# amathislab/HOISDF

Hardware: AMD Instinct MI355X
Metric: samples/sec (img + 2048 SDF queries) fwd+bwd at 1/2/4/8 MI355X (higher is better)
Workload: dtype f32 (emulated contractions, f32 accumulate, f16x2 form: operands as scaled hi + lo f16 pieces x 3 products - 22 operand bits, one power-of-two scale per ROW of a linear layer's row operand, per (sample, head) of the attention operands, per weight matrix; the attention backward's dS as three pieces x

## Files before the change

hoisdf_amd/csrc/attention_emu.h:

```cpp
#pragma once
#include "common.h"

namespace hoisdf {
namespace emu_attn {

typedef float f32x16 __attribute__((ext_vector_type(16)));
typedef float f32x4 __attribute__((ext_vector_type(4)));
typedef float f32x2 __attribute__((ext_vector_type(2)));
typedef __bf16 bf16x8 __attribute__((ext_vector_type(8)));
typedef __bf16 bf16x4 __attribute__((ext_vector_type(4)));
typedef __bf16 bf16x2 __attribute__((ext_vector_type(2)));
typedef _Float16 f16x8 __attribute__((ext_vector_type(8)));
typedef _Float16 f16x2 __attribute__((ext_vector_type(2)));
typedef unsigned int u32x4 __attribute__((ext_vector_type(4)));
typedef unsigned int u32x2 __attribute__((ext_vector_type(2)));
typedef short s16x4 __attribute__((ext_vector_type(4)));

constexpr int D = 64;
constexpr float LN2 = 0.6931471805599453f;

struct EmuAttn {
  const __bf16 *q[3];
  const __bf16 *k[3];
  const __bf16 *v[3], *vt[3];
  const __bf16 *d[3];
  const float* lse_in; const float* delta;
  float* out; float* lse; float* dq_part; float* dk; float* dv;
  int ldo, ldk, ldv;
  int B, H, Lq, Lk, Lqp, Lkp, kv_len;
  float drop_p, inv_keep;
  uint32_t thresh;
  uint64_t seed;
  const uint32_t *q_hm, *k_hm, *v_hm, *d_hm;
  float* dq_scale;
  uint32_t* mag;
};

__device__ __forceinline__ bool emu_block(int nx, int nbh, int& tile, int& bh) {
  const int L = blockIdx.x, slot = L >> 3;
  bh = (slot / nx) * 8 + (L & 7);
  tile = slot % nx;
  return bh < nbh;
}

}

int attention_bwd4_emu_launch(const emu_attn::EmuAttn& a, hipStream_t st);
int attention_bwd4h_emu_launch(const emu_attn::EmuAttn& a, hipStream_t st);
}
```

hoisdf_amd/csrc/attention_emu.hip:

```cpp
#include "attention_emu.h"

namespace hoisdf {
using namespace emu_attn;

namespace {
constexpr int RP = 72;
constexpr int TPH = 36;
constexpr int ROWS_T = 32 * RP;
constexpr int TRN_T = 64 * TPH;
constexpr float QS2 = 0.125f * 1.4426950408889634f;
#define CR(r, h) (((r) & 3) + 8 * ((r) >> 2) + 4 * (h))
#define MB(a, b, c) __builtin_amdgcn_mfma_f32_32x32x16_bf16((a), (b), (c), 0, 0, 0)
#define MB6(acc, x0, x1, x2, y0, y1, y2) \
  do {                                   \
    acc = MB(x2, y0, acc);               \
    acc = MB(x0, y2, acc);               \
    acc = MB(x1, y1, acc);               \
    acc = MB(x1, y0, acc);               \
    acc = MB(x0, y1, acc);               \
    acc = MB(x0, y0, acc);               \
  } while (0)

#define SPLIT1(x, i)                             \
  do {                                           \
// ... 505 lines not shown
  HOISDF_REQUIRE(workspace_bytes >= need, HOISDF_ERR_WORKSPACE, "attention_fwd_bf16x2: workspace %ld < %ld bytes", workspace_bytes, need);
  hipStream_t st = as_stream(stream);
  __bf16* w = reinterpret_cast<__bf16*>(workspace);
  const QkvPlaneSet s = carve_qkv(w, B, H, Lq, Lk, false, true, 2);
  if (int rc = convert_qkv(q, ldq, k, ldk, v, ldv, B, H, Lq, Lk, s, st)) return rc;
  EmuAttn a = emu_args(B, H, Lq, Lk, kv_len, 0.f, 0);
  for (int i = 0; i < 2; ++i) { a.q[i] = s.q.r[i]; a.k[i] = s.k.r[i]; a.vt[i] = s.v.t[i]; }
  a.out = o; a.lse = nullptr; a.ldo = ldo;
  const dim3 fgrid(cdiv(Lq, 128) * 8 * cdiv(B * H, 8));
  hipLaunchKernelGGL((emu_attn_fwd2_kernel<false, 2, false>), fgrid, dim3(256), 0, st, a);
  return check_launch("attention_fwd_bf16x2");
}

void hoisdf::attention_emu_plane_targets(void* workspace, int B, int H, int Lq, int Lk, int keep, QkvPlanes& qp, QkvPlanes& kvp) {
  const QkvPlaneSet s = fwd_planes(workspace, B, H, Lq, Lk, keep);
  qp = QkvPlanes{}; kvp = QkvPlanes{};
  qp.on = kvp.on = 1; qp.H = kvp.H = H; qp.E = kvp.E = H * 64; qp.qscale = kvp.qscale = QS2;
  qp.L = Lq; qp.Lp = (int)pad128(Lq); kvp.L = Lk; kvp.Lp = (int)pad128(Lk);
  for (int i = 0; i < 3; ++i) {
    qp.r[0][i] = s.q.r[i];
    kvp.r[1][i] = s.k.r[i]; kvp.r[2][i] = s.v.r[i]; kvp.vt[i] = s.v.t[i];
    if (Lq == Lk) { kvp.r[0][i] = s.q.r[i]; qp.r[1][i] = s.k.r[i]; qp.r[2][i] = s.v.r[i]; qp.vt[i] = s.v.t[i]; }
  }
}

int hoisdf::attention_fwd_emu_planes(float* o, int ldo, float* lse, int B, int H, int Lq, int Lk, int kv_len, float drop_p,
                                     uint64_t seed, void* workspace, int keep, void* stream, uint32_t* o_mag) {
  HOISDF_REQUIRE(o && workspace && ldo >= H * 64 && (ldo & 3) == 0 && (((uintptr_t)o | (uintptr_t)workspace) & 15) == 0 && B > 0 &&
                     H > 0 && Lq > 0 && Lk > 0 && kv_len > 0 && kv_len <= Lk && drop_p >= 0.f && drop_p < 1.f,
                 HOISDF_ERR_INVALID, "attention_fwd_emu_planes: bad arguments");
  return fwd_over_planes(o, ldo, lse, B, H, Lq, Lk, kv_len, drop_p, seed, workspace, keep, as_stream(stream), o_mag);
}

extern "C" long hoisdf_attention_bwd_emu_workspace(int B, int H, int Lq, int Lk, int kept) {
  if (B <= 0 || H <= 0 || Lq <= 0 || Lk <= 0) return 0;
  const size_t q = plane_elems(B, H, pad128(Lq)), k = plane_elems(B, H, pad128(Lk));
  size_t bytes = 3 * q * sizeof(__bf16) + (size_t)cdiv(Lk, 128) * B * H * Lq * 64 * sizeof(float);
  if (!kept) bytes += (3 * q + 6 * k) * sizeof(__bf16);
  return (long)bytes;
}

extern "C" int hoisdf_attention_bwd_emu(const float* q, int ldq, const float* k, int ldk, const float* v, int ldv, const float* o,
                                        int ldo, const float* dout, int lddo, const float* lse, float* delta, float* dq, float* dk,
                                        float* dv, int B, int H, int Lq, int Lk, int kv_len, float drop_p, uint64_t seed,
                                        const void* fwd_workspace, void* workspace, long workspace_bytes, void* stream) {
  return attention_bwd_emu_mag(q, ldq, k, ldk, v, ldv, o, ldo, dout, lddo, lse, delta, dq, dk, dv, B, H, Lq, Lk, kv_len, drop_p, seed,
                               fwd_workspace, workspace, workspace_bytes, nullptr, stream, nullptr, nullptr, nullptr, nullptr);
}
extern "C" int hoisdf_attention_bwd_emu_mag(const float* q, int ldq, const float* k, int ldk, const float* v, int ldv, const float* o,
                                            int ldo, const float* dout, int lddo, const float* lse, float* delta, float* dq, float* dk,
                                            float* dv, int B, int H, int Lq, int Lk, int kv_len, float drop_p, uint64_t seed,
                                            const void* fwd_workspace, void* workspace, long workspace_bytes, const uint32_t* q_mag,
                                            const uint32_t* k_mag, const uint32_t* v_mag, const uint32_t* do_mag, uint32_t* g_mag, void* stream) {
  HOISDF_REQUIRE(q_mag && k_mag && v_mag && do_mag, HOISDF_ERR_INVALID, "attention_bwd_emu_mag: the head magnitudes of q, k, v and of dout are required");
  return attention_bwd_emu_mag(q, ldq, k, ldk, v, ldv, o, ldo, dout, lddo, lse, delta, dq, dk, dv, B, H, Lq, Lk, kv_len, drop_p, seed,
                               fwd_workspace, workspace, workspace_bytes, g_mag, stream, q_mag, k_mag, v_mag, do_mag);
}
int hoisdf::attention_bwd_emu_mag(const float* q, int ldq, const float* k, int ldk, const float* v, int ldv, const float* o, int ldo,
                                  const float* dout, int lddo, const float* lse, float* delta, float* dq, float* dk, float* dv, int B,
                                  int H, int Lq, int Lk, int kv_len, float drop_p, uint64_t seed, const void* fwd_workspace,
                                  void* workspace, long workspace_bytes, uint32_t* g_mag, void* stream, const uint32_t* q_hm,
                                  const uint32_t* k_hm, const uint32_t* v_hm, const uint32_t* do_hm) {
  const bool h2 = q_hm && k_hm && v_hm && do_hm;
  HOISDF_REQUIRE(h2 || (!q_hm && !k_hm && !v_hm && !do_hm), HOISDF_ERR_INVALID, "attention_bwd_emu: head magnitudes of all of q, k, v, dout or of none");
  HOISDF_REQUIRE(!g_mag || Lq == Lk, HOISDF_ERR_INVALID, "attention_bwd_emu: one row-magnitude array for dq, dk, dv needs Lq == Lk");
  HOISDF_REQUIRE(!h2 || drop_p < 0.75f, HOISDF_ERR_INVALID, "attention_bwd_emu (f16x2 form): drop_p = %f, must be below 0.75 (as in the forward)", drop_p);
  if (int rc = check_emu(fwd_workspace && !q ? o : q, fwd_workspace && !k ? o : k, fwd_workspace && !v ? o : v, ldq, ldk, ldv, B, H, Lq,
                         Lk, kv_len, drop_p, "attention_bwd_emu")) return rc;
  HOISDF_REQUIRE(o && dout && lse && delta && dq && dk && dv && workspace, HOISDF_ERR_INVALID, "attention_bwd_emu: null pointer");
  HOISDF_REQUIRE(ldo >= H * 64 && lddo >= H * 64 && ((ldo | lddo) & 3) == 0 &&
                     (((uintptr_t)o | (uintptr_t)dout | (uintptr_t)dq | (uintptr_t)dk | (uintptr_t)dv | (uintptr_t)workspace |
                       (uintptr_t)fwd_workspace) & 15) == 0,
                 HOISDF_ERR_INVALID, "attention_bwd_emu: bad leading dims / alignment");
  const long need = hoisdf_attention_bwd_emu_workspace(B, H, Lq, Lk, fwd_workspace ? 1 : 0);
  HOISDF_REQUIRE(workspace_bytes >= need, HOISDF_ERR_WORKSPACE, "attention_bwd_emu: workspace %ld < %ld bytes", workspace_bytes, need);
  hipStream_t st = as_stream(stream);
  __bf16* w = reinterpret_cast<__bf16*>(workspace);
  const Planes pd = carve(w, plane_elems(B, H, pad128(Lq)), true, false);
  float* part = reinterpret_cast<float*>(w);
  w += (size_t)cdiv(Lk, 128) * B * H * Lq * 64 * 2;
  QkvPlaneSet s;
  if (fwd_workspace) {
    __bf16* f = reinterpret_cast<__bf16*>(const_cast<void*>(fwd_workspace));
    s = carve_qkv(f, B, H, Lq, Lk, true, true);
  } else {
    s = carve_qkv(w, B, H, Lq, Lk, true, false);
    if (int rc = convert_qkv(q, ldq, k, ldk, v, ldv, B, H, Lq, Lk, s, st, q_hm, k_hm, v_hm)) return rc;
  }
  if (int rc = convert(dout, lddo, Lq, (int)pad128(Lq), B, H, 1.f, pd, st, do_hm)) return rc;
  const long ng = (long)B * Lq * H;
  hipLaunchKernelGGL(emu_attn_delta_kernel, dim3((unsigned)((ng * 16 + 255) / 256)), dim3(256), 0, st, o, ldo, dout, lddo, delta, B, H, Lq);
  if (int rc = check_launch("attention_emu_delta")) return rc;
  EmuAttn a = emu_args(B, H, Lq, Lk, kv_len, drop_p, seed);
  for (int i = 0; i < 3; ++i) { a.q[i] = s.q.r[i]; a.k[i] = s.k.r[i]; a.v[i] = s.v.r[i]; a.d[i] = pd.r[i]; }
  a.lse_in = lse; a.delta = delta; a.dq_part = part; a.dk = dk; a.dv = dv; a.ldk = ldk; a.ldv = ldv; a.mag = g_mag;
  if (h2) {
    a.q_hm = q_hm; a.k_hm = k_hm; a.v_hm = v_hm; a.d_hm = do_hm;
    a.dq_scale = reinterpret_cast<float*>(pd.r[2]);
  }
  if (int rc = h2 ? attention_bwd4h_emu_launch(a, st) : attention_bwd4_emu_launch(a, st)) return rc;
  const long n4 = (long)B * H * Lq * 16;
  hipLaunchKernelGGL(emu_attn_dq_reduce_kernel, dim3((unsigned)((n4 + 255) / 256)), dim3(256), 0, st, part, cdiv(kv_len, 128), dq, ldq,
                     B, H, Lq, g_mag, (const float*)(h2 ? a.dq_scale : nullptr));
  return check_launch("attention_bwd_emu dq reduce");
}
```

hoisdf_amd/csrc/attention_emu_bwd4.inc:

```

namespace hoisdf {
namespace {
constexpr int NPL = B4_NPL;
constexpr int QD_PLANE = 32 * 64;
constexpr int QD_BUF = 2 * NPL * QD_PLANE;
constexpr int TT_PLANE = 128 * 32;
constexpr int TT_BUF = 3 * TT_PLANE;
constexpr int X_BUF = 2 * 32 * 64;
constexpr int TT0 = 3 * QD_BUF;
constexpr int X0_BYTES = (3 * QD_BUF + 2 * TT_BUF) * 2;
constexpr int ST0_BYTES = X0_BYTES + 2 * X_BUF * 4;
constexpr unsigned B4_LDS_BYTES = ST0_BYTES + 3 * 64 * 4;

__device__ __forceinline__ int qd_swz(int r) { return ((r >> 1) & 3) | ((((r >> 1) ^ (r >> 3)) & 1) << 2); }
__device__ __forceinline__ int qd_off(int r, int ch) { return r * 64 + ((ch ^ qd_swz(r)) << 3); }

__device__ __forceinline__ bf16x8 tr8(const __bf16* lo, const __bf16* hi) {
  const s16x4 x = __builtin_amdgcn_ds_read_tr16_b64_v4i16((s16x4 __attribute__((address_space(3)))*)(lo));
  const s16x4 y = __builtin_amdgcn_ds_read_tr16_b64_v4i16((s16x4 __attribute__((address_space(3)))*)(hi));
  return __builtin_bit_cast(bf16x8, __builtin_shufflevector(x, y, 0, 1, 2, 3, 4, 5, 6, 7));
}
}

template <bool DROP>
__global__ __launch_bounds__(256, 1) void B4_KERNEL(EmuAttn a) {
  extern __shared__ __attribute__((aligned(16))) __bf16 lds[];
  float* const xbuf = reinterpret_cast<float*>(reinterpret_cast<char*>(lds) + X0_BYTES);
  float* const stats = reinterpret_cast<float*>(reinterpret_cast<char*>(lds) + ST0_BYTES);
  const int tid = threadIdx.x, lane = tid & 63, wave = tid >> 6;
  const int c = lane & 31, h = lane >> 5, jq = lane & 15, b1 = (jq >> 3) & 1;
  int ktile, bh;
  const int nkb = (a.Lk + 127) / 128;
  if (!emu_block(nkb, a.B * a.H, ktile, bh)) return;
  const int b = bh / a.H, head = bh - b * a.H;
  const int key = ktile * 128 + wave * 32 + c;
  const bool kvalid = key < a.kv_len;
  const int nq = ktile * 128 < a.kv_len ? (a.Lq + 31) / 32 : 0;
  const int dhalf = wave & 1, khalf = wave >> 1;
  B4_SCALES

  bf16x8 kf[4][NPL], vf[4][NPL], ktf[4][NPL];
  {
    const size_t ro = ((size_t)bh * a.Lkp + key) * D;
#pragma unroll
    for (int p = 0; p < NPL; ++p)
#pragma unroll
      for (int j = 0; j < 4; ++j) {
        kf[j][p] = *reinterpret_cast<const bf16x8*>(a.k[p] + ro + 16 * j + 8 * h);
        vf[j][p] = *reinterpret_cast<const bf16x8*>(a.v[p] + ro + 16 * j + 8 * h);
      }
    const size_t ko = ((size_t)bh * a.Lkp + ktile * 128 + 64 * khalf + 8 * h) * D + 32 * dhalf + c;
#pragma unroll
    for (int p = 0; p < NPL; ++p)
#pragma unroll
      for (int ks = 0; ks < 4; ++ks) {
        bf16x8 t;
#pragma unroll
        for (int i = 0; i < 8; ++i)
          t[i] = ktile * 128 + 64 * khalf + 16 * ks + 8 * h + i < a.kv_len ? a.k[p][ko + (size_t)(16 * ks + i) * D] : (__bf16)0.f;
        ktf[ks][p] = t;
      }
  }
#pragma unroll
  for (int p = 0; p < NPL; ++p)
#pragma unroll
    for (int j = 0; j < 4; ++j) {
      asm volatile("" : "+a"(kf[j][p]));
// ... 16 lines not shown
#pragma unroll
    for (int e = 0; e < 2; ++e) trb[e] = (4 * h + (jq >> 2)) * 64 + ((e ^ b1) << 5) + (low2 << 3) + (jq & 1) * 4;
  }
  int tqb[2];
#pragma unroll
  for (int s2 = 0; s2 < 2; ++s2) {
    const int kr = 64 * khalf + 8 * h + 4 * s2 + (jq >> 2);
    tqb[s2] = kr * 32 + (((4 * (c >> 4) + (jq & 3)) ^ ((kr >> 1) & 7)) << 2);
  }
  const int tw0 = (32 * wave + c) * 32 + ((h ^ ((c >> 1) & 7)) << 2);
  const int xw0 = khalf * 2048 + c * 64 + (8 * dhalf << 2) + ((h ^ (c & 7)) << 2);
  const int xr0 = (8 * wave + (lane >> 4)) * 64 + (((lane & 15) ^ (lane >> 4)) << 2);
  const int xr1 = (xr0 + 256) ^ 16;
  const int st_o = qd_off(tid >> 3, tid & 7);

  u32x4 sg[2 * NPL];
  float rstat = 0.f;
  const size_t rowbase = (size_t)bh * a.Lqp * D;
  const __bf16* const qb0 = a.q[0] + rowbase; const __bf16* const qb1 = a.q[1] + rowbase; const __bf16* const qb2 = a.q[2] + rowbase;
  const __bf16* const db0 = a.d[0] + rowbase; const __bf16* const db1 = a.d[1] + rowbase; const __bf16* const db2 = a.d[2] + rowbase;
  unsigned goff = (unsigned)((tid >> 3) * D + (tid & 7) * 8);
  const float* const stat_src = (tid < 32 ? a.lse_in : a.delta) + (size_t)bh * a.Lq;
#define B4_LOADP(i_) do { sg[i_] = *reinterpret_cast<const u32x4*>(((i_) == 0 ? qb0 : (i_) == 1 ? qb1 : (i_) == NPL ? db0 : (i_) == NPL + 1 ? db1 : (i_) == 2 ? qb2 : db2) + goff); } while (0)
#define B4_LOADS(QT_, GHOST_)                                                                                          \
  do {                                                                                                                 \
    if (tid < 64) {                                                                                                    \
      const int q_ = (QT_) * 32 + (tid & 31);                                                                          \
      rstat = (q_ < a.Lq && !(GHOST_)) ? stat_src[q_] : (tid < 32 ? INFINITY : 0.f);                                   \
    }                                                                                                                  \
  } while (0)
#define B4_STOREP(i_, BUF_) do { *reinterpret_cast<u32x4*>(lds + (BUF_) + (i_) * QD_PLANE + st_o) = sg[i_]; } while (0)
#define B4_STORES(SB_) do { if (tid < 64) stats[(SB_) + tid] = rstat; } while (0)

  float* const part = a.dq_part + ((size_t)ktile * a.B * a.H + bh) * a.Lq * D;
  if (nq > 0) {
#pragma unroll
    for (int pt = 0; pt < 2; ++pt) {
      const int qt = min(pt, nq - 1);
      goff = (unsigned)(qt * 32 * D + (tid >> 3) * D + (tid & 7) * 8);
#pragma unroll
      for (int i = 0; i < 2 * NPL; ++i) B4_LOADP(i);
      B4_LOADS(qt, pt >= nq);
#pragma unroll
      for (int i = 0; i < 2 * NPL; ++i) B4_STOREP(i, pt * QD_BUF);
      B4_STORES(pt * 64);
    }
    int qt_next = min(2, nq - 1);
    goff = (unsigned)(qt_next * 32 * D + (tid >> 3) * D + (tid & 7) * 8);
#pragma unroll
    for (int i = 0; i < 2 * NPL; ++i) B4_LOADP(i);
    B4_LOADS(qt_next, 2 >= nq);
    __syncthreads();

    int qd_cur = 0, qd_nxt = QD_BUF, qd_fre = 2 * QD_BUF;
    int st_cur = 0, st_nxt = 64, st_fre = 128;
    int tt_w = TT0, tt_r = TT0 + TT_BUF;
    int x_a = 0, x_b = X_BUF;
    uint32_t hb = 0;
    const uint32_t dthr = a.thresh & 0xffff0000u;
    const int hsh = (key & 1) ? 0 : 16;
    B4_FORM_STATE
    if (DROP) hb = drop_rowkey(a.seed, (uint32_t)(bh * a.Lq + 4 * h)) + (uint32_t)(key >> 1) * 0x9E3779B9U + B4_HB_PAIR;

    f32x16 s, dp, dq;
    f32x4 xo0[2], xo1[2];
    bf16x8 fr[2][NPL];
    u32x4 pwv[NPL][2], gwv[3][2];
    f32x2 pe[8], pd[8], xx[8], ff[8];
    float dsc[16], lq[16], dl[16];
#pragma unroll
    for (int r = 0; r < 16; ++r) dsc[r] = 1.f;
#pragma unroll
    for (int p = 0; p < 3; ++p)
#pragma unroll
      for (int i = 0; i < 2; ++i) { if (p < NPL) pwv[p][i] = u32x4{0u, 0u, 0u, 0u}; gwv[p][i] = u32x4{0u, 0u, 0u, 0u}; }

#define MFMA_SP(acc_, a_, b_) asm volatile(B4_MFMA " %0, %1, %2, %0" : "+v"(acc_) : "v"(a_), "a"(b_))
#define MFMA_SP0(acc_, a_, b_) asm volatile(B4_MFMA " %0, %1, %2, 0" : "=&v"(acc_) : "v"(a_), "a"(b_))
#define MFMA_Q(acc_, a_, b_) asm volatile(B4_MFMA " %0, %1, %2, %0" : "+v"(acc_) : "a"(a_), "v"(b_))
#define MFMA_Q0(acc_, a_, b_) asm volatile(B4_MFMA " %0, %1, %2, 0" : "=&v"(acc_) : "a"(a_), "v"(b_))
#define MFMA_VK(acc_, a_, b_) asm volatile(B4_MFMA " %0, %1, %2, %0" : "+a"(acc_) : "v"(a_), "v"(b_))
#define FRQ(p_, j_) (*reinterpret_cast<const bf16x8*>(lds + qd_cur + aoff[j_] + (p_) * QD_PLANE))
#define FRD(p_, j_) (*reinterpret_cast<const bf16x8*>(lds + qd_cur + aoff[j_] + (NPL + (p_)) * QD_PLANE))
#define FRQN(p_, j_) (*reinterpret_cast<const bf16x8*>(lds + qd_nxt + aoff[j_] + (p_) * QD_PLANE))
#define FRDN(p_, j_) (*reinterpret_cast<const bf16x8*>(lds + qd_nxt + aoff[j_] + (NPL + (p_)) * QD_PLANE))
#define FRA(pl_, jj_, mt_) tr8(lds + qd_cur + trb[(mt_)] + (pl_) * QD_PLANE + (16 * (jj_)) * 64, \
                               lds + qd_cur + trb[(mt_) ^ 1] + (pl_) * QD_PLANE + (16 * (jj_) + 8) * 64)
#define FRT(p_, ks_) tr8(lds + tt_r + tqb[0] + (p_) * TT_PLANE + (16 * (ks_)) * 32, lds + tt_r + tqb[1] + (p_) * TT_PLANE + (16 * (ks_)) * 32)
#define PWF(p_, jj_) __builtin_bit_cast(bf16x8, pwv[p_][jj_])
#define GWF(p_, jj_) __builtin_bit_cast(bf16x8, gwv[p_][jj_])
#define PIN2(x_) asm volatile("" : "+v"(x_))
#define XOL(i_)                                                                                                        \
  do {                                                                                                                 \
    xo0[i_] = *reinterpret_cast<const f32x4*>(xbuf + x_a + ((i_) ? xr1 : xr0));                                        \
    xo1[i_] = *reinterpret_cast<const f32x4*>(xbuf + x_a + 2048 + ((i_) ? xr1 : xr0));                                 \
  } while (0)
#define XOS(i_)                                                                                                        \
  do {                                                                                                                 \
    const int q_ = (t - 2) * 32 + 8 * wave + 4 * (i_) + (lane >> 4);                                                   \
    if (t >= 2 && q_ < a.Lq) *reinterpret_cast<f32x4*>(part + (unsigned)(q_ * D + 4 * (lane & 15))) = xo0[i_] + xo1[i_]; \
  } while (0)
#define CRC(r_) (((r_) & 3) + 8 * ((r_) >> 2))
#define PB(q_)                                                                                                         \
  do {                                                                                                                 \
    _Pragma("unroll") for (int i_ = 0; i_ < 2; ++i_) {                                                                 \
      const int m_ = 2 * (q_) + i_;                                                                                    \
      pd[m_] = DROP ? f32x2{pe[m_].x * dsc[2 * m_], pe[m_].y * dsc[2 * m_ + 1]} : pe[m_];                              \
      const uint32_t w_ = cvt2(pd[m_]);                                                                                \
      pwv[0][m_ >> 2][m_ & 3] = w_;                                                                                    \
      PIN2(pwv[0][m_ >> 2][m_ & 3]);                                                                                   \
    }                                                                                                                  \
  } while (0)
#define PC(q_)                                                                                                         \
  do {                                                                                                                 \
    _Pragma("unroll") for (int i_ = 0; i_ < 2; ++i_) {                                                                 \
      const int m_ = 2 * (q_) + i_;                                                                                    \
      xx[m_] = pd[m_] - unpack2(pwv[0][m_ >> 2][m_ & 3]);                                                              \
      PIN2(xx[m_]);                                                                                                    \
    }                                                                                                                  \
  } while (0)
#define QB(q_)                                                                                                         \
  do {                                                                                                                 \
    _Pragma("unroll") for (int i_ = 0; i_ < 2; ++i_) {                                                                 \
      const int m_ = 2 * (q_) + i_;                                                                                    \
      xx[m_] = xx[m_] - unpack2(gwv[0][m_ >> 2][m_ & 3]);                                                              \
      PIN2(xx[m_]);                                                                                                    \
    }                                                                                                                  \
  } while (0)
#define QC(q_)                                                                                                         \
  do {                                                                                                                 \
    _Pragma("unroll") for (int i_ = 0; i_ < 2; ++i_) {                                                                 \
      const int m_ = 2 * (q_) + i_;                                                                                    \
      const uint32_t w_ = cvt2(xx[m_]);                                                                                \
// ... 33 lines not shown
      B4_ITER();
      { const int t_ = qd_cur; qd_cur = qd_nxt; qd_nxt = qd_fre; qd_fre = t_; }
      { const int t_ = st_cur; st_cur = st_nxt; st_nxt = st_fre; st_fre = t_; }
      { const int t_ = tt_w; tt_w = tt_r; tt_r = t_; }
      { const int t_ = x_a; x_a = x_b; x_b = t_; }
      __syncthreads();
    }
    {
      const int t = nq + 1;
      XOL(0); XOL(1);
      XOS(0); XOS(1);
    }
  }
  uint32_t gmax = 0u;
  if (key < a.Lk) {
    float* pk = a.dk + ((size_t)b * a.Lk + key) * a.ldk + head * D;
    float* pv = a.dv + ((size_t)b * a.Lk + key) * a.ldv + head * D;
#pragma unroll
    for (int mt = 0; mt < 2; ++mt)
#pragma unroll
      for (int g = 0; g < 4; ++g) {
        const float zk = kvalid ? dk_scale : 0.f, zv = kvalid ? dv_scale : 0.f;
        const float4 gk = make_float4(dk[mt][4 * g] * zk, dk[mt][4 * g + 1] * zk, dk[mt][4 * g + 2] * zk, dk[mt][4 * g + 3] * zk);
        const float4 gv = make_float4(dv[mt][4 * g] * zv, dv[mt][4 * g + 1] * zv, dv[mt][4 * g + 2] * zv, dv[mt][4 * g + 3] * zv);
        *reinterpret_cast<float4*>(pk + 32 * mt + 8 * g + 4 * h) = gk;
        *reinterpret_cast<float4*>(pv + 32 * mt + 8 * g + 4 * h) = gv;
        gmax = max(gmax, max(mag_bits4(gk), mag_bits4(gv)));
      }
  }
  if (a.mag) {
    gmax = max(gmax, (uint32_t)__shfl_xor((int)gmax, 32, 64));
    if (h == 0 && key < a.Lk) atomicMax(a.mag + (size_t)b * a.Lk + key, gmax);
  }
}

int B4_LAUNCH(const EmuAttn& a, hipStream_t st) {
  static bool attr_set = false;
  if (!attr_set) {
    const void* ks[2] = {reinterpret_cast<const void*>(B4_KERNEL<true>), reinterpret_cast<const void*>(B4_KERNEL<false>)};
    for (const void* k : ks)
      if (hipFuncSetAttribute(k, hipFuncAttributeMaxDynamicSharedMemorySize, (int)B4_LDS_BYTES) != hipSuccess) {
        set_error("attention_bwd_emu" B4_WHO ": cannot raise the dynamic LDS limit to %u bytes", B4_LDS_BYTES);
        return HOISDF_ERR_LAUNCH;
      }
    attr_set = true;
  }
  const dim3 grid(cdiv(a.Lk, 128) * 8 * cdiv(a.B * a.H, 8));
  if (a.drop_p > 0.f) hipLaunchKernelGGL((B4_KERNEL<true>), grid, dim3(256), B4_LDS_BYTES, st, a);
  else hipLaunchKernelGGL((B4_KERNEL<false>), grid, dim3(256), B4_LDS_BYTES, st, a);
  return check_launch("attention_bwd_emu (" B4_TAG ")");
}

}
```

hoisdf_amd/csrc/attn_bwd4_phase.inc:

```
#define BWD4_ITER()                                                                \
  do {                                                                             \
    MFMA_SP0(s, fr[0][0], kf[0][2]); XOL(0); SB();                                 \
    MFMA_SP(s, fr[0][2], kf[0][0]); fr[1][0] = FRQ(0, 1); XOL(1); SB();            \
    MFMA_SP(s, fr[0][1], kf[0][1]); fr[1][1] = FRQ(1, 1); SB();                    \
    MFMA_SP(s, fr[0][0], kf[0][1]); fr[1][2] = FRQ(2, 1); SB();                    \
    MFMA_SP(s, fr[0][1], kf[0][0]); STQ(0); SB();                                  \
    MFMA_SP(s, fr[0][0], kf[0][0]); STQ(1); SB();                                  \
    MFMA_SP(s, fr[1][0], kf[1][2]); STQ(2); SB();                                  \
    MFMA_SP(s, fr[1][2], kf[1][0]); fr[0][0] = FRQ(0, 2); SB();                    \
    MFMA_SP(s, fr[1][1], kf[1][1]); fr[0][1] = FRQ(1, 2); SB();                    \
    MFMA_SP(s, fr[1][0], kf[1][1]); fr[0][2] = FRQ(2, 2); SB();                    \
    MFMA_SP(s, fr[1][1], kf[1][0]); STQ(3); SB();                                  \
    MFMA_SP(s, fr[1][0], kf[1][0]); STQ(4); SB();                                  \
    MFMA_SP(s, fr[0][0], kf[2][2]); STQ(5); SB();                                  \
    MFMA_SP(s, fr[0][2], kf[2][0]); fr[1][0] = FRQ(0, 3); SB();                    \
    MFMA_SP(s, fr[0][1], kf[2][1]); fr[1][1] = FRQ(1, 3); SB();                    \
    MFMA_SP(s, fr[0][0], kf[2][1]); fr[1][2] = FRQ(2, 3); SB();                    \
    MFMA_SP(s, fr[0][1], kf[2][0]); STS(); SB();                                   \
    MFMA_SP(s, fr[0][0], kf[2][0]); LDG(0); SB();                                  \
    MFMA_SP(s, fr[1][0], kf[3][2]); LDG(1); SB();                                  \
    MFMA_SP(s, fr[1][2], kf[3][0]); fr[0][0] = FRD(0, 0); SB();                    \
    MFMA_SP(s, fr[1][1], kf[3][1]); fr[0][1] = FRD(1, 0); LQ(0); SB();             \
    MFMA_SP(s, fr[1][0], kf[3][1]); fr[0][2] = FRD(2, 0); LQ(1); SB();             \
    MFMA_SP(s, fr[1][1], kf[3][0]); LDG(2); SB();                                  \
    MFMA_SP(s, fr[1][0], kf[3][0]); LDG(3); SB();                                  \
    MFMA_SP0(dp, fr[0][2], vf[0][0]); LDG(4); SB();                                \
    MFMA_SP(dp, fr[0][0], vf[0][2]); fr[1][0] = FRD(0, 1); LQ(2); LQ(3); SB();     \
    MFMA_SP(dp, fr[0][1], vf[0][1]); fr[1][1] = FRD(1, 1); SB();                   \
    MFMA_SP(dp, fr[0][1], vf[0][0]); fr[1][2] = FRD(2, 1); SB();                   \
    MFMA_SP(dp, fr[0][0], vf[0][1]); LDG(5); SB();                                 \
    MFMA_SP(dp, fr[0][0], vf[0][0]); LDS_(); SB();                                 \
    MFMA_SP(dp, fr[1][2], vf[1][0]); PA(0); SB();                                  \
    MFMA_SP(dp, fr[1][0], vf[1][2]); fr[0][0] = FRD(0, 2); SB();                   \
    MFMA_SP(dp, fr[1][1], vf[1][1]); fr[0][1] = FRD(1, 2); SB();                   \
    MFMA_SP(dp, fr[1][1], vf[1][0]); fr[0][2] = FRD(2, 2); SB();                   \
    MFMA_SP(dp, fr[1][0], vf[1][1]); PA(1); SB();                                  \
    MFMA_SP(dp, fr[1][0], vf[1][0]); PB(0); SB();                                  \
    MFMA_SP(dp, fr[0][2], vf[2][0]); PB(1); SB();                                  \
    MFMA_SP(dp, fr[0][0], vf[2][2]); fr[1][0] = FRD(0, 3); SB();                   \
    MFMA_SP(dp, fr[0][1], vf[2][1]); fr[1][1] = FRD(1, 3); SB();                   \
    MFMA_SP(dp, fr[0][1], vf[2][0]); fr[1][2] = FRD(2, 3); SB();                   \
    MFMA_SP(dp, fr[0][0], vf[2][1]); PC(0); SB();                                  \
    MFMA_SP(dp, fr[0][0], vf[2][0]); XOS(0); SB();                                 \
    MFMA_SP(dp, fr[1][2], vf[3][0]); XOS(1); SB();                                 \
    MFMA_SP(dp, fr[1][0], vf[3][2]); fq0[0] = FRT(0, 0); SB();                     \
    MFMA_SP(dp, fr[1][1], vf[3][1]); fr[0][1] = FRT(1, 0); DL(0); SB();            \
    MFMA_SP(dp, fr[1][1], vf[3][0]); fr[0][2] = FRT(2, 0); DL(1); SB();            \
    MFMA_SP(dp, fr[1][0], vf[3][1]); PC(1); SB();                                  \
    MFMA_SP(dp, fr[1][0], vf[3][0]); PD(0); SB();                                  \
    MFMA_Q0(dq, ktf[0][2], fq0[0]); PD(1); SB();                                   \
    MFMA_Q(dq, ktf[0][0], fr[0][2]); fq0[1] = FRT(0, 1); DL(2); DL(3); SB();       \
    MFMA_Q(dq, ktf[0][1], fr[0][1]); fr[1][1] = FRT(1, 1); SB();                   \
    MFMA_Q(dq, ktf[0][1], fq0[0]); fr[1][2] = FRT(2, 1); SB();                     \
    MFMA_Q(dq, ktf[0][0], fr[0][1]); PE(0); SB();                                  \
    MFMA_Q(dq, ktf[1][2], fq0[1]); PE(1); SB();                                    \
    MFMA_Q(dq, ktf[1][0], fr[1][2]); fq0[2] = FRT(0, 2); QA(0); SB();              \
    MFMA_Q(dq, ktf[1][1], fr[1][1]); fr[0][1] = FRT(1, 2); QA(1); SB();            \
    MFMA_Q(dq, ktf[1][1], fq0[1]); fr[0][2] = FRT(2, 2); QB(0); SB();              \
    MFMA_Q(dq, ktf[1][0], fr[1][1]); PA(2); SB();                                  \
    MFMA_Q(dq, ktf[2][2], fq0[2]); PA(3); SB();                                    \
    MFMA_Q(dq, ktf[2][0], fr[0][2]); fq0[3] = FRT(0, 3); QB(1); SB();              \
    MFMA_Q(dq, ktf[2][1], fr[0][1]); fr[1][1] = FRT(1, 3); QC(0); SB();            \
    MFMA_Q(dq, ktf[2][1], fq0[2]); fr[1][2] = FRT(2, 3); QC(1); SB();              \
    MFMA_Q(dq, ktf[2][0], fr[0][1]); PB(2); SB();                                  \
    MFMA_Q(dq, ktf[3][2], fq0[3]); PB(3); SB();                                    \
    MFMA_Q(dq, ktf[3][0], fr[1][2]); PC(2); QD(0); SB();                           \
    MFMA_Q(dq, ktf[3][1], fr[1][1]); PC(3); SB();                                  \
    MFMA_Q(dq, ktf[3][1], fq0[3]); PD(2); SB();                                    \
    MFMA_Q(dq, ktf[3][0], fr[1][1]); PD(3); SB();                                  \
    MFMA_Q(dq, ktf[0][0], fq0[0]); fr[0][0] = FRA(3 + 0, 0, 0); PE(2); SB();       \
    MFMA_Q(dq, ktf[1][0], fq0[1]); fr[0][1] = FRA(3 + 1, 0, 0); PE(3); SB();       \
    MFMA_Q(dq, ktf[2][0], fq0[2]); fr[0][2] = FRA(3 + 2, 0, 0); SB();              \
    MFMA_Q(dq, ktf[3][0], fq0[3]); QD(1); SB();                                    \
    MFMA_VK(dv[0], fr[0][2], PWF(0, 0)); TW(0); SB();                              \
    MFMA_VK(dv[0], fr[0][0], PWF(2, 0)); fr[1][0] = FRA(3 + 0, 0, 1); SB();        \
    MFMA_VK(dv[0], fr[0][1], PWF(1, 0)); fr[1][1] = FRA(3 + 1, 0, 1); XW(0); SB(); \
    MFMA_VK(dv[0], fr[0][1], PWF(0, 0)); fr[1][2] = FRA(3 + 2, 0, 1); XW(1); SB(); \
// ... 46 lines not shown
```

hoisdf_amd/csrc/attn_bwd4h_phase.inc:

```
#define BWD4H_ITER()                                                                          \
  do {                                                                                        \
    MFMA_SP0(s, fr[0][0], kf[0][1]); XOL(0); SB();                                            \
    MFMA_SP(s, fr[0][1], kf[0][0]); fr[1][0] = FRQ(0, 1); XOL(1); SB();                       \
    MFMA_SP(s, fr[0][0], kf[0][0]); fr[1][1] = FRQ(1, 1); SB();                               \
    MFMA_SP(s, fr[1][0], kf[1][1]); STQ(0); SB();                                             \
    MFMA_SP(s, fr[1][1], kf[1][0]); fr[0][0] = FRQ(0, 2); SB();                               \
    MFMA_SP(s, fr[1][0], kf[1][0]); fr[0][1] = FRQ(1, 2); SB();                               \
    MFMA_SP(s, fr[0][0], kf[2][1]); STQ(1); SB();                                             \
    MFMA_SP(s, fr[0][1], kf[2][0]); fr[1][0] = FRQ(0, 3); STQ(2); SB();                       \
    MFMA_SP(s, fr[0][0], kf[2][0]); fr[1][1] = FRQ(1, 3); LQ(0); SB();                        \
    MFMA_SP(s, fr[1][0], kf[3][1]); fr[0][0] = FRD(0, 0); LQ(1); SB();                        \
    MFMA_SP(s, fr[1][1], kf[3][0]); fr[0][1] = FRD(1, 0); LQ(2); LQ(3); SB();                 \
    MFMA_SP(s, fr[1][0], kf[3][0]); STQ(3); STS(); SB();                                      \
    MFMA_SP0(dp, fr[0][1], vf[0][0]); ft[0][0] = FRT(0, 0); LDG(0); SB();                     \
    MFMA_SP(dp, fr[0][0], vf[0][1]); fr[1][0] = FRD(0, 1); ft[0][1] = FRT(1, 0); SB();        \
    MFMA_SP(dp, fr[0][0], vf[0][0]); fr[1][1] = FRD(1, 1); ft[0][2] = FRT(2, 0); PA(0); SB(); \
    MFMA_SP(dp, fr[1][1], vf[1][0]); ft[1][0] = FRT(0, 1); LDG(1); SB();                      \
    MFMA_SP(dp, fr[1][0], vf[1][1]); fr[0][0] = FRD(0, 2); ft[1][1] = FRT(1, 1); PA(1); SB(); \
    MFMA_SP(dp, fr[1][0], vf[1][0]); fr[0][1] = FRD(1, 2); ft[1][2] = FRT(2, 1); PB(0); SB(); \
    MFMA_SP(dp, fr[0][1], vf[2][0]); ft[2][0] = FRT(0, 2); LDG(2); SB();                      \
    MFMA_SP(dp, fr[0][0], vf[2][1]); fr[1][0] = FRD(0, 3); ft[2][1] = FRT(1, 2); PB(1); SB(); \
    MFMA_SP(dp, fr[0][0], vf[2][0]); fr[1][1] = FRD(1, 3); ft[2][2] = FRT(2, 2); SB();        \
    MFMA_SP(dp, fr[1][1], vf[3][0]); ft[3][0] = FRT(0, 3); LDG(3); SB();                      \
    MFMA_SP(dp, fr[1][0], vf[3][1]); ft[3][1] = FRT(1, 3); LDS_(); SB();                      \
    MFMA_SP(dp, fr[1][0], vf[3][0]); ft[3][2] = FRT(2, 3); DL(0); SB();                       \
    MFMA_Q0(dq, ktf[0][1], ft[0][1]); PC(0); DL(1); DL(2); DL(3); SB();                       \
    MFMA_Q(dq, ktf[0][0], ft[0][2]); XOS(0); SB();                                            \
    MFMA_Q(dq, ktf[0][1], ft[0][0]); fr[0][0] = FRA(2 + 0, 0, 0); SB();                       \
    MFMA_Q(dq, ktf[0][0], ft[0][1]); fr[0][1] = FRA(2 + 1, 0, 0); SB();                       \
    MFMA_Q(dq, ktf[1][1], ft[1][1]); XOS(1); SB();                                            \
    MFMA_Q(dq, ktf[1][0], ft[1][2]); PC(1); SB();                                             \
    MFMA_Q(dq, ktf[1][1], ft[1][0]); PD(0); SB();                                             \
    MFMA_Q(dq, ktf[1][0], ft[1][1]); PD(1); QA(0); SB();                                      \
    MFMA_Q(dq, ktf[2][1], ft[2][1]); PA(2); SB();                                             \
    MFMA_Q(dq, ktf[2][0], ft[2][2]); PA(3); SB();                                             \
    MFMA_Q(dq, ktf[2][1], ft[2][0]); PB(2); SB();                                             \
    MFMA_Q(dq, ktf[2][0], ft[2][1]); PB(3); SB();                                             \
    MFMA_Q(dq, ktf[3][1], ft[3][1]); PC(2); QA(1); SB();                                      \
    MFMA_Q(dq, ktf[3][0], ft[3][2]); PC(3); QB(0); SB();                                      \
    MFMA_Q(dq, ktf[3][1], ft[3][0]); PD(2); QB(1); SB();                                      \
    MFMA_Q(dq, ktf[3][0], ft[3][1]); PD(3); QC(0); SB();                                      \
    MFMA_Q(dq, ktf[0][0], ft[0][0]); QC(1); SB();                                             \
    MFMA_Q(dq, ktf[1][0], ft[1][0]); QD(0); SB();                                             \
    MFMA_Q(dq, ktf[2][0], ft[2][0]); QD(1); SB();                                             \
    MFMA_Q(dq, ktf[3][0], ft[3][0]); TW(0); SB();                                             \
    MFMA_VK(dv[0], fr[0][1], PWF(0, 0)); TW(1); SB();                                         \
    MFMA_VK(dv[0], fr[0][0], PWF(1, 0)); fr[1][0] = FRA(2 + 0, 0, 1); QA(2); SB();            \
    MFMA_VK(dv[0], fr[0][0], PWF(0, 0)); fr[1][1] = FRA(2 + 1, 0, 1); QA(3); SB();            \
    MFMA_VK(dv[1], fr[1][1], PWF(0, 0)); QB(2); XW(0); SB();                                  \
    MFMA_VK(dv[1], fr[1][0], PWF(1, 0)); fr[0][0] = FRA(2 + 0, 1, 0); QB(3); SB();            \
    MFMA_VK(dv[1], fr[1][0], PWF(0, 0)); fr[0][1] = FRA(2 + 1, 1, 0); QC(2); SB();            \
    MFMA_VK(dv[0], fr[0][1], PWF(0, 1)); QC(3); XW(1); SB();                                  \
    MFMA_VK(dv[0], fr[0][0], PWF(1, 1)); fr[1][0] = FRA(2 + 0, 1, 1); QD(2); XW(2); SB();     \
    MFMA_VK(dv[0], fr[0][0], PWF(0, 1)); fr[1][1] = FRA(2 + 1, 1, 1); QD(3); SB();            \
    MFMA_VK(dv[1], fr[1][1], PWF(0, 1)); fr[0][0] = FRA(0, 0, 0); TW(2); SB();                \
    MFMA_VK(dv[1], fr[1][0], PWF(1, 1)); fr[0][1] = FRA(1, 0, 0); TW(3); SB();                \
    MFMA_VK(dv[1], fr[1][0], PWF(0, 1)); XW(3); SB();                                         \
    MFMA_VK(dk[0], fr[0][1], GWF(1, 0)); SB();                                                \
    MFMA_VK(dk[0], fr[0][0], GWF(2, 0)); fr[1][0] = FRA(0, 0, 1); SB();                       \
    MFMA_VK(dk[0], fr[0][1], GWF(0, 0)); fr[1][1] = FRA(1, 0, 1); SB();                       \
    MFMA_VK(dk[0], fr[0][0], GWF(1, 0)); HA(0); SB();                                         \
    MFMA_VK(dk[0], fr[0][0], GWF(0, 0)); HA(1); SB();                                         \
    MFMA_VK(dk[1], fr[1][1], GWF(1, 0)); HB(0); SB();                                         \
// ... 16 lines not shown
```

include/hoisdf.h:

```cpp
#ifndef HOISDF_H_
#define HOISDF_H_

#include <stdint.h>

#ifdef __cplusplus
extern "C" {
#endif

#define HOISDF_VERSION_MAJOR 0
#define HOISDF_VERSION_MINOR 1

typedef enum hoisdf_status {
  HOISDF_OK = 0,
  HOISDF_ERR_INVALID = -1,
  HOISDF_ERR_LAUNCH = -2,
  HOISDF_ERR_TOO_FEW = -3,
  HOISDF_ERR_WORKSPACE = -4
} hoisdf_status;

#define HOISDF_MAX_LEVELS 8

typedef struct hoisdf_pyramid {
  int n_levels;
  int B;
  const float* data[HOISDF_MAX_LEVELS];
  int C[HOISDF_MAX_LEVELS];
  int H[HOISDF_MAX_LEVELS];
  int W[HOISDF_MAX_LEVELS];
} hoisdf_pyramid;

typedef struct hoisdf_pyramid_grad {
  int n_levels;
  int B;
  float* data[HOISDF_MAX_LEVELS];
  int C[HOISDF_MAX_LEVELS];
  int H[HOISDF_MAX_LEVELS];
  int W[HOISDF_MAX_LEVELS];
} hoisdf_pyramid_grad;

const char* hoisdf_version(void);
const char* hoisdf_last_error(void);
void hoisdf_set_deterministic(int on);
void hoisdf_set_gemm_emu(int on);
int hoisdf_get_gemm_emu(void);
int hoisdf_get_deterministic(void);

int hoisdf_project_gather_fwd(const hoisdf_pyramid* pyr, const float* points,
                              const int32_t* sample_idx, long n_rows, int rows_per_sample,
                              const float* center, const float* cam_intr, float scale,
                              int img_h, int img_w, float* feat, int ldf, float* cam_out,
                              float* uv_out, void* stream);
int hoisdf_project_gather_bwd(const hoisdf_pyramid_grad* dpyr, const float* points,
                              const int32_t* sample_idx, long n_rows, int rows_per_sample,
                              const float* center, const float* cam_intr, float scale,
                              int img_h, int img_w, const float* dfeat, int ldf, void* stream);

int hoisdf_linear_fwd(const float* x, int ldx, const float* W, int ldw, const float* bias,
                      float* y, int ldy, long M, int N, int K, int act, float drop_p,
                      uint64_t seed, uint32_t* relu_bits, void* stream);
int hoisdf_linear_bwd_input(const float* dy, int lddy, const uint32_t* relu_bits, float drop_p,
                            const float* W, int ldw, float* dx, int lddx, long M, int N, int K,
                            int accumulate ,
                            void* stream);
long hoisdf_linear_bwd_weight_workspace(long M, int N, int K);
int hoisdf_linear_bwd_weight(const float* dy, int lddy, const uint32_t* relu_bits, float drop_p,
                             const float* x, int ldx, float* dW, int lddw, float* db, long M, int N,
                             int K, float* workspace, long workspace_floats, void* stream);
long hoisdf_linear_emu_image_bytes(int rows, int K);
int hoisdf_linear_emu_prepare(const float* W, int ldw, int N, int K, int transpose, void* image, void* stream);
typedef struct hoisdf_emu_prep_item {
  const float* W;
  void* image;
  long first_block;
  int ldw, N, K, transpose;
} hoisdf_emu_prep_item;
long hoisdf_linear_emu_prepare_blocks(int N, int K, int transpose);
int hoisdf_linear_emu_prepare_batch(const hoisdf_emu_prep_item* d_items, int n, long total_blocks, void* stream);
int hoisdf_linear_emu_supported(const float* a, long lda, int contraction);
// ... 517 lines not shown
```

Measured before the change: 450.0.

## Group key tiles per attention-backward block to shrink dq partial buffers

Each attention-backward block now loops over a group of 1, 2, 4 or 8 key tiles instead of handling a single one. It accumulates its dq partials in place by reading back the previous pass's values, so the partial workspace and the dq reduce kernel scale with the number of key groups rather than key tiles. By default the group size is picked from the shape so that at least 512 blocks remain, and a setter lets callers override it. The intent is to cut global write and read traffic for dq partials and the reduce cost, at the price of fewer blocks, serialized passes and an extra load in each pass.

Result: no change. 452.1 (median of 6 runs) (+0.5%).

```diff
diff --git a/hoisdf_amd/csrc/attention_emu.h b/hoisdf_amd/csrc/attention_emu.h
--- a/hoisdf_amd/csrc/attention_emu.h
+++ b/hoisdf_amd/csrc/attention_emu.h
@@ -28,6 +28,7 @@
   float* out; float* lse; float* dq_part; float* dk; float* dv;
   int ldo, ldk, ldv;
   int B, H, Lq, Lk, Lqp, Lkp, kv_len;
+  int key_group;
   float drop_p, inv_keep;
   uint32_t thresh;
   uint64_t seed;
@@ -45,6 +46,8 @@
 
 }
 
+int attention_bwd_key_group(int B, int H, int Lk);
+
 int attention_bwd4_emu_launch(const emu_attn::EmuAttn& a, hipStream_t st);
 int attention_bwd4h_emu_launch(const emu_attn::EmuAttn& a, hipStream_t st);
 }
diff --git a/hoisdf_amd/csrc/attention_emu.hip b/hoisdf_amd/csrc/attention_emu.hip
--- a/hoisdf_amd/csrc/attention_emu.hip
+++ b/hoisdf_amd/csrc/attention_emu.hip
@@ -561,10 +561,24 @@
   return fwd_over_planes(o, ldo, lse, B, H, Lq, Lk, kv_len, drop_p, seed, workspace, keep, as_stream(stream), o_mag);
 }
 
+namespace { int g_bwd_key_group = 0; }
+extern "C" void hoisdf_set_attention_bwd_key_group(int tiles) {
+  if (tiles == 0 || tiles == 1 || tiles == 2 || tiles == 4 || tiles == 8) g_bwd_key_group = tiles;
+  else set_error("set_attention_bwd_key_group: %d refused (0 = by shape, or 1, 2, 4, 8); the setting stays %d", tiles, g_bwd_key_group);
+}
+extern "C" int hoisdf_get_attention_bwd_key_group(void) { return g_bwd_key_group; }
+int hoisdf::attention_bwd_key_group(int B, int H, int Lk) {
+  if (g_bwd_key_group) return g_bwd_key_group;
+  for (int t = 4; t > 1; t >>= 1)
+    if ((long)B * H * cdiv(cdiv(Lk, 128), t) >= 512) return t;
+  return 1;
+}
+
 extern "C" long hoisdf_attention_bwd_emu_workspace(int B, int H, int Lq, int Lk, int kept) {
   if (B <= 0 || H <= 0 || Lq <= 0 || Lk <= 0) return 0;
   const size_t q = plane_elems(B, H, pad128(Lq)), k = plane_elems(B, H, pad128(Lk));
-  size_t bytes = 3 * q * sizeof(__bf16) + (size_t)cdiv(Lk, 128) * B * H * Lq * 64 * sizeof(float);
+  const int groups = cdiv(cdiv(Lk, 128), attention_bwd_key_group(B, H, Lk));
+  size_t bytes = 3 * q * sizeof(__bf16) + (size_t)groups * B * H * Lq * 64 * sizeof(float);
   if (!kept) bytes += (3 * q + 6 * k) * sizeof(__bf16);
   return (long)bytes;
 }
@@ -607,7 +621,8 @@
   __bf16* w = reinterpret_cast<__bf16*>(workspace);
   const Planes pd = carve(w, plane_elems(B, H, pad128(Lq)), true, false);
   float* part = reinterpret_cast<float*>(w);
-  w += (size_t)cdiv(Lk, 128) * B * H * Lq * 64 * 2;
+  const int key_group = attention_bwd_key_group(B, H, Lk);
+  w += (size_t)cdiv(cdiv(Lk, 128), key_group) * B * H * Lq * 64 * 2;
   QkvPlaneSet s;
   if (fwd_workspace) {
     __bf16* f = reinterpret_cast<__bf16*>(const_cast<void*>(fwd_workspace));
@@ -623,13 +638,14 @@
   EmuAttn a = emu_args(B, H, Lq, Lk, kv_len, drop_p, seed);
   for (int i = 0; i < 3; ++i) { a.q[i] = s.q.r[i]; a.k[i] = s.k.r[i]; a.v[i] = s.v.r[i]; a.d[i] = pd.r[i]; }
   a.lse_in = lse; a.delta = delta; a.dq_part = part; a.dk = dk; a.dv = dv; a.ldk = ldk; a.ldv = ldv; a.mag = g_mag;
+  a.key_group = key_group;
   if (h2) {
     a.q_hm = q_hm; a.k_hm = k_hm; a.v_hm = v_hm; a.d_hm = do_hm;
     a.dq_scale = reinterpret_cast<float*>(pd.r[2]);
   }
   if (int rc = h2 ? attention_bwd4h_emu_launch(a, st) : attention_bwd4_emu_launch(a, st)) return rc;
   const long n4 = (long)B * H * Lq * 16;
-  hipLaunchKernelGGL(emu_attn_dq_reduce_kernel, dim3((unsigned)((n4 + 255) / 256)), dim3(256), 0, st, part, cdiv(kv_len, 128), dq, ldq,
-                     B, H, Lq, g_mag, (const float*)(h2 ? a.dq_scale : nullptr));
+  hipLaunchKernelGGL(emu_attn_dq_reduce_kernel, dim3((unsigned)((n4 + 255) / 256)), dim3(256), 0, st, part, cdiv(cdiv(kv_len, 128), key_group),
+                     dq, ldq, B, H, Lq, g_mag, (const float*)(h2 ? a.dq_scale : nullptr));
   return check_launch("attention_bwd_emu dq reduce");
 }
diff --git a/hoisdf_amd/csrc/attention_emu_bwd4.inc b/hoisdf_amd/csrc/attention_emu_bwd4.inc
--- a/hoisdf_amd/csrc/attention_emu_bwd4.inc
+++ b/hoisdf_amd/csrc/attention_emu_bwd4.inc
@@ -27,12 +27,18 @@
   extern __shared__ __attribute__((aligned(16))) __bf16 lds[];
   float* const xbuf = reinterpret_cast<float*>(reinterpret_cast<char*>(lds) + X0_BYTES);
   float* const stats = reinterpret_cast<float*>(reinterpret_cast<char*>(lds) + ST0_BYTES);
-  const int tid = threadIdx.x, lane = tid & 63, wave = tid >> 6;
+  int group, bh_;
+  const int nkb = (a.Lk + 127) / 128;
+  if (!emu_block((nkb + a.key_group - 1) / a.key_group, a.B * a.H, group, bh_)) return;
+  for (int pass = 0; pass < a.key_group && group * a.key_group + pass < nkb; ++pass) {
+  int tid = threadIdx.x, bh = bh_;
+  asm volatile("" : "+v"(tid), "+s"(bh));
+  const int lane = tid & 63, wave = tid >> 6;
   const int c = lane & 31, h = lane >> 5, jq = lane & 15, b1 = (jq >> 3) & 1;
-  int ktile, bh;
-  const int nkb = (a.Lk + 127) / 128;
-  if (!emu_block(nkb, a.B * a.H, ktile, bh)) return;
   const int b = bh / a.H, head = bh - b * a.H;
+  float* const part = a.dq_part + ((size_t)group * a.B * a.H + bh) * a.Lq * D;
+  const int ktile = group * a.key_group + pass;
+  const bool add = pass > 0;
   const int key = ktile * 128 + wave * 32 + c;
   const bool kvalid = key < a.kv_len;
   const int nq = ktile * 128 < a.kv_len ? (a.Lq + 31) / 32 : 0;
@@ -115,7 +121,6 @@
 #define B4_STOREP(i_, BUF_) do { *reinterpret_cast<u32x4*>(lds + (BUF_) + (i_) * QD_PLANE + st_o) = sg[i_]; } while (0)
 #define B4_STORES(SB_) do { if (tid < 64) stats[(SB_) + tid] = rstat; } while (0)
 
-  float* const part = a.dq_part + ((size_t)ktile * a.B * a.H + bh) * a.Lq * D;
   if (nq > 0) {
 #pragma unroll
     for (int pt = 0; pt < 2; ++pt) {
@@ -146,7 +151,7 @@
     if (DROP) hb = drop_rowkey(a.seed, (uint32_t)(bh * a.Lq + 4 * h)) + (uint32_t)(key >> 1) * 0x9E3779B9U + B4_HB_PAIR;
 
     f32x16 s, dp, dq;
-    f32x4 xo0[2], xo1[2];
+    f32x4 xo0[2], xo1[2], xp[2] = {f32x4{0.f, 0.f, 0.f, 0.f}, f32x4{0.f, 0.f, 0.f, 0.f}};
     bf16x8 fr[2][NPL];
     u32x4 pwv[NPL][2], gwv[3][2];
     f32x2 pe[8], pd[8], xx[8], ff[8];
@@ -181,7 +186,15 @@
 #define XOS(i_)                                                                                                        \
   do {                                                                                                                 \
     const int q_ = (t - 2) * 32 + 8 * wave + 4 * (i_) + (lane >> 4);                                                   \
-    if (t >= 2 && q_ < a.Lq) *reinterpret_cast<f32x4*>(part + (unsigned)(q_ * D + 4 * (lane & 15))) = xo0[i_] + xo1[i_]; \
+    if (t >= 2 && q_ < a.Lq) {                                                                                         \
+      const f32x4 v_ = xo0[i_] + xo1[i_];                                                                              \
+      *reinterpret_cast<f32x4*>(part + (unsigned)(q_ * D + 4 * (lane & 15))) = add ? xp[i_] + v_ : v_;                 \
+    }                                                                                                                  \
+  } while (0)
+#define XPL(i_)                                                                                                        \
+  do {                                                                                                                 \
+    const int q_ = (t - 1) * 32 + 8 * wave + 4 * (i_) + (lane >> 4);                                                   \
+    if (add && t >= 1 && q_ < a.Lq) xp[i_] = *reinterpret_cast<const f32x4*>(part + (unsigned)(q_ * D + 4 * (lane & 15))); \
   } while (0)
 #define CRC(r_) (((r_) & 3) + 8 * ((r_) >> 2))
 #define PB(q_)                                                                                                         \
@@ -281,6 +294,7 @@
     gmax = max(gmax, (uint32_t)__shfl_xor((int)gmax, 32, 64));
     if (h == 0 && key < a.Lk) atomicMax(a.mag + (size_t)b * a.Lk + key, gmax);
   }
+  }
 }
 
 int B4_LAUNCH(const EmuAttn& a, hipStream_t st) {
@@ -294,7 +308,7 @@
       }
     attr_set = true;
   }
-  const dim3 grid(cdiv(a.Lk, 128) * 8 * cdiv(a.B * a.H, 8));
+  const dim3 grid(cdiv(cdiv(a.Lk, 128), a.key_group) * 8 * cdiv(a.B * a.H, 8));
   if (a.drop_p > 0.f) hipLaunchKernelGGL((B4_KERNEL<true>), grid, dim3(256), B4_LDS_BYTES, st, a);
   else hipLaunchKernelGGL((B4_KERNEL<false>), grid, dim3(256), B4_LDS_BYTES, st, a);
   return check_launch("attention_bwd_emu (" B4_TAG ")");
diff --git a/hoisdf_amd/csrc/attn_bwd4_phase.inc b/hoisdf_amd/csrc/attn_bwd4_phase.inc
--- a/hoisdf_amd/csrc/attn_bwd4_phase.inc
+++ b/hoisdf_amd/csrc/attn_bwd4_phase.inc
@@ -41,8 +41,8 @@
     MFMA_SP(dp, fr[0][1], vf[2][1]); fr[1][1] = FRD(1, 3); SB();                   \
     MFMA_SP(dp, fr[0][1], vf[2][0]); fr[1][2] = FRD(2, 3); SB();                   \
     MFMA_SP(dp, fr[0][0], vf[2][1]); PC(0); SB();                                  \
-    MFMA_SP(dp, fr[0][0], vf[2][0]); XOS(0); SB();                                 \
-    MFMA_SP(dp, fr[1][2], vf[3][0]); XOS(1); SB();                                 \
+    MFMA_SP(dp, fr[0][0], vf[2][0]); XOS(0); XPL(0); SB();                         \
+    MFMA_SP(dp, fr[1][2], vf[3][0]); XOS(1); XPL(1); SB();                         \
     MFMA_SP(dp, fr[1][0], vf[3][2]); fq0[0] = FRT(0, 0); SB();                     \
     MFMA_SP(dp, fr[1][1], vf[3][1]); fr[0][1] = FRT(1, 0); DL(0); SB();            \
     MFMA_SP(dp, fr[1][1], vf[3][0]); fr[0][2] = FRT(2, 0); DL(1); SB();            \
diff --git a/hoisdf_amd/csrc/attn_bwd4h_phase.inc b/hoisdf_amd/csrc/attn_bwd4h_phase.inc
--- a/hoisdf_amd/csrc/attn_bwd4h_phase.inc
+++ b/hoisdf_amd/csrc/attn_bwd4h_phase.inc
@@ -25,10 +25,10 @@
     MFMA_SP(dp, fr[1][0], vf[3][1]); ft[3][1] = FRT(1, 3); LDS_(); SB();                      \
     MFMA_SP(dp, fr[1][0], vf[3][0]); ft[3][2] = FRT(2, 3); DL(0); SB();                       \
     MFMA_Q0(dq, ktf[0][1], ft[0][1]); PC(0); DL(1); DL(2); DL(3); SB();                       \
-    MFMA_Q(dq, ktf[0][0], ft[0][2]); XOS(0); SB();                                            \
+    MFMA_Q(dq, ktf[0][0], ft[0][2]); XOS(0); XPL(0); SB();                                    \
     MFMA_Q(dq, ktf[0][1], ft[0][0]); fr[0][0] = FRA(2 + 0, 0, 0); SB();                       \
     MFMA_Q(dq, ktf[0][0], ft[0][1]); fr[0][1] = FRA(2 + 1, 0, 0); SB();                       \
-    MFMA_Q(dq, ktf[1][1], ft[1][1]); XOS(1); SB();                                            \
+    MFMA_Q(dq, ktf[1][1], ft[1][1]); XOS(1); XPL(1); SB();                                    \
     MFMA_Q(dq, ktf[1][0], ft[1][2]); PC(1); SB();                                             \
     MFMA_Q(dq, ktf[1][1], ft[1][0]); PD(0); SB();                                             \
     MFMA_Q(dq, ktf[1][0], ft[1][1]); PD(1); QA(0); SB();                                      \
diff --git a/include/hoisdf.h b/include/hoisdf.h
--- a/include/hoisdf.h
+++ b/include/hoisdf.h
@@ -44,6 +44,8 @@
 void hoisdf_set_gemm_emu(int on);
 int hoisdf_get_gemm_emu(void);
 int hoisdf_get_deterministic(void);
+void hoisdf_set_attention_bwd_key_group(int tiles);
+int hoisdf_get_attention_bwd_key_group(void);
 
 int hoisdf_project_gather_fwd(const hoisdf_pyramid* pyr, const float* points,
                               const int32_t* sample_idx, long n_rows, int rows_per_sample,
```
